# QitaoZhao/ContextAware-PoseFormer

Hardware: AMD Instinct MI355X
Metric: frames/sec (higher is better)
Workload: dtype f32; 1 GPU; configs[1]: batch 64/GPU hrnet_32 256x256 image + 17 kpts -> 17x3, PoseFormer lifter embed 128 levels 4, fp32 tensors, fp32 accumulation; 3x3 stride-1 convs from batch 5: each operand as two fp16 pieces under exact power-of-two block scales (to 2^-23), three piece products on the 16-bit matrix pipe -- same measured distance to fp64 as the direct fp32 MFMA kernel; Inf / NaN / |x| >= 1.5e23 give NaN; frames_per_gpu=64, parallelism=dp1 (independent frames, no collective), plan_flags=0

## Files before the change

contextaware-poseformer_amd/csrc/engine.cpp:

```cpp
#include <stdio.h>
#include <string.h>

#include <algorithm>
#include <vector>

#include "engine.h"

namespace capf {

#define HIP_TRY(expr)                                                                      \
    do {                                                                                   \
        hipError_t _e = (expr);                                                            \
        if (_e != hipSuccess) {                                                            \
            err = std::string(#expr) + ": " + hipGetErrorString(_e);                       \
            return CAPF_ERR_HIP;                                                           \
        }                                                                                  \
    } while (0)

Engine::ConvSrc Engine::conv_src(const Pack& pk) const {
    return {params[pk.w[0]].ptr, params[pk.bn.g].ptr, params[pk.bn.b].ptr, params[pk.bn.m].ptr, params[pk.bn.v].ptr, 1e-5f};
}

int Engine::repack(hipStream_t s, bool lifter_only) {
    for (const Param& p : params) {
// ... 20 lines not shown
        float* B = pack_arena + pk.b_off;
        if (pk.kind == CONV_BN) {
            if (lifter_only) continue;
            const ConvSrc c = conv_src(pk);
            if (pk.bf16) {
                HIP_TRY(launch_pack_conv_bf16(c.w, c.g, c.b, c.m, c.v, c.eps, W, B, pk.N, pk.Cin, pk.ks, pk.Kpad, s, f16()));
                if (pk.rh) HIP_TRY(launch_pack_conv_bf16_rh(c.w, c.g, c.b, c.m, c.v, c.eps, pack_arena + pk.rh_off, B, pk.N, pk.Cin, bf16_rh_width(pk.Cin), s, f16()));
                if (pk.ws) HIP_TRY(launch_pack_conv_bf16_ws(c.w, c.g, c.b, c.m, c.v, c.eps, pack_arena + pk.ws_off, B, pk.N, pk.Cin, s, f16()));
            } else if (pk.fast3x3) {
                if (!pk.wino_skip) HIP_TRY(launch_pack_conv_wino(c.w, c.g, c.b, c.m, c.v, c.eps, W, B, pk.N, pk.Cin, s, pk.Kpad == 18 * pk.Cin ? 43 : 23));
                HIP_TRY(launch_pack_conv(c.w, c.g, c.b, c.m, c.v, c.eps, pack_arena + pk.direct_off, B, pk.N, pk.Cin, pk.ks, pk.direct_Kpad, s));
                if (pk.x3)
                    HIP_TRY((plan.x3_h2 ? launch_pack_conv_f32h2 : launch_pack_conv_f32x3)(c.w, c.g, c.b, c.m, c.v, c.eps, pack_arena + pk.x3_off, B, pk.N, pk.Cin, s));
            } else {
                HIP_TRY(launch_pack_conv(c.w, c.g, c.b, c.m, c.v, c.eps, W, B, pk.N, pk.Cin, pk.ks, pk.Kpad, s));
            }
            continue;
        }
        int n0 = 0;
        for (int i = 0; i < pk.n_lin; ++i) {
            const int n = (int)params[pk.w[i]].shape[0];
            const float* w = params[pk.w[i]].ptr;
            if (pk.bf16)
                HIP_TRY(launch_pack_conv_bf16(w, nullptr, nullptr, nullptr, nullptr, 0.f, reinterpret_cast<unsigned short*>(W) + (size_t)n0 * pk.Kpad,
                                              nullptr, n, pk.K, 1, pk.Kpad, s, f16()));
            else if (pk.quad) HIP_TRY(launch_pack_linear_quad(w, W, n, pk.K, n0, pk.N, s));
            else HIP_TRY(launch_pack_linear(w, W + (size_t)n0 * pk.Kpad, n, pk.K, pk.Kpad, s));
            jobs.push_back(CopySegment{params[pk.b[i]].ptr, B + n0, n, 0});
            n0 += n;
        }
// ... 36 lines not shown
    GemmArgs a{};
    a.A = op.in[0] == -2 ? images : ptr(op.in[0]);
    if (pk.in_place) {
        a.Wp = params[pk.w[0]].ptr;
        a.bias = params[pk.b[0]].ptr;
    } else {
        a.Wp = pack_arena + pk.w_off;
        a.bias = pack_arena + pk.b_off;
    }
    a.res = op.res_param >= 0 ? params[op.res_param].ptr : ptr(op.aux);
    a.out = ptr(op.out);
    a.M = (int)(op.rows_per_frame * batch);
    a.N = op.N; a.K = op.K; a.Kpad = pk.Kpad;
    if (pk.rh) a.Wp2 = pack_arena + pk.rh_off;
    if (pk.ws || pk.x3) a.Wp3 = pack_arena + (pk.ws ? pk.ws_off : pk.x3_off);
    a.x3_h2 = pk.x3 && plan.x3_h2;
    if (a.x3_h2 && op.h2_utab >= 0 && utab_on_device) a.h2_utab = reinterpret_cast<const unsigned*>(pack_arena + utab_off) + op.h2_utab;
    const Family family = gemm_family(op, batch);
    if (pk.h2g && batch >= H2G_MIN_BATCH && family == Family::F32 && !op.pw_pair) a.Wh2 = pack_arena + pk.h2g_off;
    if (op.fast3x3 && family == Family::F32) {
        a.Wp = pack_arena + pk.direct_off;
        a.Kpad = pk.direct_Kpad;
    } else if (family == Family::F32_TILE && pk.wino_skip) {
        a.Wp = nullptr;
    }
    a.conv = op.conv;
    a.Cin = op.Cin; a.H = op.H; a.W = op.W; a.Ho = op.Ho; a.Wo = op.Wo;
    a.ks = op.ks; a.stride = op.stride; a.pad = op.pad;
    a.amap = op.amap; a.omap = op.omap; a.rmap = op.rmap;
    a.act = op.act;
// ... 18 lines not shown
        a.split_cnt = on_side_chain ? split_cnt_side : split_cnt;
        a.split_ws_elems = SPLIT_WS_ELEMS; a.split_cnt_elems = SPLIT_CNT_ELEMS;
    }
    if (op.ln.w >= 0) {
        a.ln_g = params[op.ln.w].ptr;
        a.ln_b = params[op.ln.b].ptr;
        a.ln_eps = op.eps;
    }
    return a;
}

Engine::FusedLaunch Engine::fused_at(int i, int batch, int last_op, bool bneck_only) const {
    const int n_all = (int)ops.size();
    if (i < 0 || i >= n_all) return {};
    const Op& o = ops[i];
    if (o.kind == OP_FORK) {
        if (!plan.use_bneck || !b16() || o.fork.lanes != 2 || o.region < 0) return {};
        const int j = regions[o.region].second;
        if (j != i + 4 || j + 1 >= last_op || j + 1 >= n_all) return {};
        int c1 = -1, c2 = -1, ds = -1;
        for (int k = i + 1; k < j; ++k) {
            const Op& g = ops[k];
            if (g.kind != OP_GEMM || !g.conv || g.bf16 != 1) return {};
            if (g.lane == 1) ds = k; else if (c1 < 0) c1 = k; else c2 = k;
        }
        const int c3 = j + 1;
        if (c1 < 0 || c2 < 0 || ds < 0 || ops[c3].kind != OP_GEMM || !ops[c3].conv || ops[c3].bf16 != 1) return {};
        if (ops[c2].in[0] != ops[c1].out || ops[ds].in[0] != ops[c1].in[0] || ops[c3].in[0] != ops[c2].out || ops[c3].aux != ops[ds].out) return {};
        if (ops[c1].rows_per_frame * batch < 65536) return {};
        if (!bneck0_bf16_ok(gemm_args(ops[c1], batch), gemm_args(ops[c2], batch), gemm_args(ops[ds], batch), gemm_args(ops[c3], batch))) return {};
// ... 6 lines not shown
                  o.rows_per_frame * batch >= 65536;
        for (const Op* g : {&o, &c2, &c3})
            ok = ok && g->kind == OP_GEMM && g->conv && g->bf16 == 1 && g->region == o.region && g->lane == o.lane && g->up_in < 0;
        if (ok && bneck1_bf16_ok(gemm_args(o, batch), gemm_args(c2, batch), gemm_args(c3, batch))) return {Fusion::BNECK1, 3, {i, i + 1, i + 2}};
    }
    if (bneck_only || !plan.use_pwchain || i + 1 >= last_op || i + 1 >= n_all) return {};
    const Op& b = ops[i + 1];
    if (!o.conv || b.kind != OP_GEMM || !b.conv || o.bf16 != b.bf16 || o.bf16 > 1 || b.in[0] != o.out || b.region != o.region || b.lane != o.lane) return {};
    if (o.bf16 && (fused_leader(i, batch, true).n || fused_at(i + 1, batch, last_op, true).n)) return {};
    const GemmArgs ga = gemm_args(o, batch), gb = gemm_args(b, batch);
    if (!(o.bf16 ? gemm_bf16_pwchain_ok(ga, gb) : gemm_f32_pwchain_ok(ga, gb))) return {};
    return {Fusion::PWCHAIN, 2, {i, i + 1}};
}

Engine::FusedLaunch Engine::fused_leader(int i, int batch, bool bneck_only) const {
    for (int f = i - 5; f <= i; ++f) {
        const FusedLaunch l = fused_at(f, batch, (int)ops.size(), bneck_only);
        for (int k = 0; k < l.n; ++k)
            if (l.m[k] == i) return l;
    }
    return {};
}

Engine::Family Engine::gemm_family(const Op& op, int batch) const {
    const bool tile = batch >= op.tile_lo && batch <= op.tile_hi;
    if (op.bf16) return op.bf16 == 2 ? Family::BF16_ROWS : tile ? Family::BF16_TILE : Family::BF16;
    if (tile) return Family::F32_TILE;
    return op.fast3x3 && batch >= plan.wino_min_batch && !packs[op.pack].wino_skip ? Family::WINO : Family::F32;
}

bool Engine::tile_takes(const Op& op, int batch) const {
// ... 160 lines not shown
            HIP_TRY(launch_mlp_chain(ptr(op.out), op.amap, (int)(op.rows_per_frame * batch), op.eps, w, s));
            break;
        }
        case OP_HEAD:
            HIP_TRY(launch_head(ptr(op.in[0]), params[op.ln.w].ptr, params[op.ln.b].ptr, op.eps, params[op.head.w].ptr,
                                params[op.head.b].ptr, out, (int)(op.rows_per_frame * batch), op.C, op.head.N, s));
            break;
        default: break;
    }
    return CAPF_OK;
}

int Engine::run_region_grouped(hipStream_t s, int batch, int region, LaunchLog* log, unsigned lane_mask) {
    auto mine = [&](const Op& op) { return ((lane_mask >> op.lane) & 1u) != 0; };
    auto groupable = [&](const Op& op, const GemmArgs& a) {
        if (op.kind != OP_GEMM) return false;
        switch (gemm_family(op, batch)) {
            case Family::BF16: return gemm_bf16_groupable(a);
            case Family::BF16_TILE: case Family::F32_TILE: return true;
            case Family::WINO: return gemm_wino_ok(a);
            case Family::F32: return gemm_f32_groupable(a);
            default: return false;
        }
    };
    for (const std::vector<int>& level : region_levels[region]) {
        for (Family pass : {Family::F32, Family::BF16_TILE, Family::BF16, Family::F32_TILE, Family::WINO}) {
            GemmArgs group[MAXG];
            int members[MAXG];
            int n = 0;
            auto flush = [&]() -> int {
                if (n == 0) return CAPF_OK;
// ... 62 lines not shown
    hipStream_t main_stream = s;
    if (plan.use_h2g && (batch >= H2G_MIN_BATCH || has_res_chain) && last_op > n_backbone_ops && !b16()) {
        const int rc = ensure_h2g_lifter(s);
        if (rc) return rc;
    }
    const bool grouped = (lanes == 2 || lanes == 3) && !ev;
    const bool par = lanes == 1 && !ev && !log && side[0];
    for (int oi = first_op; oi < last_op; ++oi) {
        const Op& op = ops[oi];
        s = (par && op.lane > 0) ? side[op.lane - 1] : main_stream;
        if (ev) HIP_TRY(hipEventRecord(ev[oi], s));
        if (const FusedLaunch f = ev ? FusedLaunch{} : fused_at(oi, batch, last_op); f.n) {
            const bool tap = debug || last_op < (int)ops.size();
            GemmArgs m[4];
            for (int k = 0; k < f.n; ++k) m[k] = gemm_args(ops[f.m[k]], batch);
            if (log) HIP_TRY(log->mark(s, f.m, f.n));
            if (f.kind == Fusion::BNECK0) HIP_TRY(launch_bneck0_bf16(m[0], m[1], m[2], m[3], tap, s));
            else if (f.kind == Fusion::BNECK1) HIP_TRY(launch_bneck1_bf16(m[0], m[1], m[2], tap, s));
            else if (op.bf16) HIP_TRY(launch_gemm_bf16_pwchain(m[0], m[1], s));
            else HIP_TRY(launch_gemm_f32_pwchain(m[0], m[1], s));
            oi = f.m[f.n - 1];
            continue;
        }
        switch (op.kind) {
            case OP_FORK: {
                if (grouped && regions[op.region].second <= last_op) {
                    const bool two = two_chains(op, batch) && !log && side[0];
                    if (two) {
                        HIP_TRY(hipEventRecord(events[op.fork.first_event], main_stream));
                        HIP_TRY(hipStreamWaitEvent(side[0], events[op.fork.first_event], 0));
// ... 884 lines not shown
    return capf::launch_keypoints_loss(pred, gt, validity, rows, dim, mode, threshold, loss, dpred,
                                       static_cast<hipStream_t>(stream)) == hipSuccess ? CAPF_OK : CAPF_ERR_HIP;
}

int capf_num_ops(const capf_handle* h) { return h ? (int)h->e.ops.size() : CAPF_ERR_INVALID; }

int capf_op_info(const capf_handle* h, int index, int batch, const char** name, const char** kernel, double* flops) {
    if (!h || index < 0 || index >= (int)h->e.ops.size() || batch <= 0) return CAPF_ERR_INVALID;
    const capf::Op& op = h->e.ops[index];
    if (name) *name = op.name.c_str();
    if (flops) *flops = op.flops_per_frame * batch;
    if (kernel) {
        const capf::Engine::FusedLaunch f = h->e.fused_leader(index, batch);
        *kernel = f.kind == capf::Engine::Fusion::BNECK0 ? capf::bneck0_bf16_kernel_name(h->e.f16())
                  : f.kind == capf::Engine::Fusion::BNECK1 ? capf::bneck1_bf16_kernel_name(h->e.f16())
                  : f.kind == capf::Engine::Fusion::PWCHAIN ? (op.bf16 ? capf::gemm_bf16_pwchain_kernel_name(h->e.f16()) : capf::gemm_f32_pwchain_kernel_name())
                  : h->e.op_route(op, batch).kernel;
    }
    return CAPF_OK;
}

int capf_op_executed_flops(const capf_handle* h, int index, int batch, double* flops) {
    if (!h || index < 0 || index >= (int)h->e.ops.size() || batch <= 0 || !flops) return CAPF_ERR_INVALID;
    *flops = h->e.op_route(h->e.ops[index], batch).flops;
    return CAPF_OK;
}

int capf_op_bytes(const capf_handle* h, int index, int batch, double* bytes) {
    if (!h || index < 0 || index >= (int)h->e.ops.size() || batch <= 0 || !bytes) return CAPF_ERR_INVALID;
    const capf::Engine& e = h->e;
    const capf::Op& op = e.ops[index];
    const double B = batch, act = op.bf16 ? 2.0 : 4.0;
    const double fact = op.feat_bf16 ? 2.0 : 4.0;
    const capf::Sampler& sm = op.smp;
    const capf::Attn& at = op.attn;
    double b = 0.0;
    switch (op.kind) {
        case capf::OP_GEMM: {
            const capf::Pack& pk = e.packs[op.pack];
            const double M = (double)op.rows_per_frame * B;
            const double in_elems = op.conv ? B * op.H * op.W * op.Cin : M * op.K;
            if (op.bf16 == 2) {
                b = in_elems * 2.0 + (double)pk.N * pk.K * 2.0 + (double)pk.N * 4.0 + M * op.N * (op.out_bf16 ? 2.0 : 4.0) +
                    (op.aux >= 0 ? M * op.N * 4.0 : 0.0);
                break;
            }
            b = in_elems * (op.conv && !op.bf16 ? 4.0 : act)
                + (double)pk.N * pk.K * (pk.bf16 ? 2.0 : 4.0) + (double)pk.N * 4.0
                + M * op.N * (op.st_f32 ? 4.0 + (op.sh >= 0 ? 2.0 : 0.0) : op.out_bf16 ? 2.0 : act)
                + ((op.aux >= 0 || op.res_param >= 0) ? M * op.N * (op.f32s ? 4.0 : act) : 0.0)
                + ((op.conv && op.up_in >= 0) ? B * op.up_H * op.up_W * op.N * act : 0.0);
            break;
        }
        case capf::OP_FUSE: {
            const double out = B * op.H * op.W * op.C;
            b = out * act + (op.sh >= 0 ? out * 2.0 : 0.0);
            for (int i = 0; i < op.n_in; ++i) b += out * act / (double)(1 << (2 * op.shift[i]));
            break;
        }
// ... 259 lines not shown
```

contextaware-poseformer_amd/csrc/engine.h:

```cpp
#pragma once
#include <hip/hip_runtime.h>
#include <stdint.h>

#include <array>
#include <map>
#include <string>
#include <vector>

#include "capf.h"
#include "kernels.h"

namespace capf {

struct Param {
    std::string name;
    int64_t shape[4] = {0, 0, 0, 0};
    int ndim = 0;
    int kind = 0;
    const float* ptr = nullptr;
    int64_t numel() const {
        int64_t n = 1;
        for (int i = 0; i < ndim; ++i) n *= shape[i];
        return n;
    }
// ... 21 lines not shown
    int n_lin = 0;
    BnRef bn;
    int N = 0, K = 0, Cin = 0, ks = 1;
    size_t w_off = 0, b_off = 0;
    int Kpad = 0;
    bool in_place = false;
    bool bf16 = false;
    bool quad = false;
    bool fast3x3 = false;
    bool wino_skip = false;
    size_t direct_off = 0; int direct_Kpad = 0;
    bool rh = false; size_t rh_off = 0; int rh_Kpad = 0;
    bool ws = false; size_t ws_off = 0;
    bool x3 = false; size_t x3_off = 0;
    bool h2g = false; size_t h2g_off = 0; int h2g_Kpad = 0;
    bool chain = false; size_t chain_off = 0;
};

struct LinearRef { int w = -1, b = -1, N = 0, K = 0; };
struct LnRef { int w = -1, b = -1; };
struct LifterMlp { LnRef norm2; LinearRef fc1, fc2; };
struct LifterAtt { LnRef norm1; LinearRef qkv, proj; LifterMlp mlp; };
struct LifterCtx {
    LnRef norm1;
    LinearRef aw, so, embed_proj[4];
    LifterMlp mlp;
    int ao_pack = -1;
    int tap_pos = -1, tap_idx = -1;
};
struct LifterSchema {
// ... 40 lines not shown
    Sampler smp;
    LinearRef coord;
    int pos = -1;
    LinearRef head;
    Attn attn;
    std::vector<ChainBlock> blocks;
    int lvlH[4] = {0, 0, 0, 0}, lvlW[4] = {0, 0, 0, 0}, lvlC[4] = {0, 0, 0, 0};
    int idx_lvl[4] = {-1, -1, -1, -1};
    int tap_pos = -1, tap_idx = -1;
    int pq[4] = {-1, -1, -1, -1};
    int pb[4] = {-1, -1, -1, -1};
    double flops_per_frame = 0.0;
    int bf16 = 0;
    int fast3x3 = 0;
    int pw_pair = 0;
    int tile_lo = 0, tile_hi = -1;
    int out_bf16 = 0;
    int h2_exps = -1, h2_role = 0, h2_peer = -1;
    long h2_utab = -1;
    int f32s = 0, st_f32 = 0, sh = -1;
    int feat_bf16 = 0;
    int bneck_c3 = -1;
    int lane = 0;
    int region = -1;
    int level = -1;
};

struct NamedTensor {
    int buf;
    int64_t shape[4];
// ... 144 lines not shown
    ConvSrc conv_src(const Pack& pk) const;
    int repack(hipStream_t s, bool lifter_only = false);
    int ensure_h2g_lifter(hipStream_t s);
    int run(hipStream_t s, int batch, int first_op, int last_op, hipEvent_t* ev = nullptr, LaunchLog* log = nullptr);
    int exec_op(const Op& op, hipStream_t s, int batch);
    bool skipped(const Op& op) const { return op.debug_only && !debug; }
    FuseSumArgs fuse_args(const Op& op, int batch) const;
    enum class Family { NONE = -1, F32, BF16, BF16_TILE, F32_TILE, WINO, BF16_ROWS };
    struct OpRoute { Family family; const char* kernel; double flops; };
    bool tile_takes(const Op& op, int batch) const;
    Family gemm_family(const Op& op, int batch) const;
    hipError_t launch_f32_tile(const GemmArgs* list, int n, hipStream_t s) const {
        return (plan.x3_h2 ? launch_gemm_f32h2_group : launch_gemm_f32x3_group)(list, n, s);
    }
    OpRoute op_route(const Op& op, int batch) const;
    enum class Fusion { NONE, BNECK0, BNECK1, PWCHAIN };
    struct FusedLaunch { Fusion kind = Fusion::NONE; int n = 0; int m[4] = {-1, -1, -1, -1}; };
    FusedLaunch fused_at(int i, int batch, int last_op, bool bneck_only = false) const;
    FusedLaunch fused_leader(int i, int batch, bool bneck_only = false) const;
    int run_region_grouped(hipStream_t s, int batch, int region, LaunchLog* log, unsigned lane_mask = ~0u);
    bool two_chains(const Op& fork_op, int batch) const { return lanes == 3 && fork_op.fork.lanes >= 2 && batch >= 16 && batch <= 128; }
    GemmArgs gemm_args(const Op& op, int batch, bool planes = true) const;

    int train_batch = 0;
    int64_t train_generation = 0;
    void invalidate_train() { train_batch = 0; ++train_generation; t_h2_base = nullptr; }
    int feat_batch = 0;
    void train_layout(int B, TrainLayout& L) const;
    size_t train_elems(int B) const;
    int forward_train(hipStream_t s, int B, const float* masks);
    int backward(hipStream_t s, int B, const float* dOut, float* flat_grad, const float* masks, float* const* dfeat = nullptr);
// ... 34 lines not shown
```

contextaware-poseformer_amd/csrc/igemm_f32_pwchain.hip:

```cpp
#include "kernels.h"

namespace capf {

typedef float f32x4 __attribute__((ext_vector_type(4)));
typedef float f32x16 __attribute__((ext_vector_type(16)));
typedef unsigned u32x4 __attribute__((ext_vector_type(4)));
typedef __amdgpu_buffer_rsrc_t rsrc_t;

template <int K1, int N1, int N2>
__global__ __launch_bounds__(256, 1) void igemm_f32_pwchain_kernel(GemmArgs p3, GemmArgs p1, int ntiles) {
#if defined(__HIP_DEVICE_COMPILE__)
    constexpr int NT1 = N1 / 32, NT2 = N2 / 32, ST1 = K1 / 8;
    constexpr int W3F = N1 * K1, W1F = N2 * N1;
    constexpr unsigned OOB = 0x80000000u;
    static_assert(K1 % 32 == 0 && N1 % 32 == 0 && N2 == 64, "whole 32-float sub-chunks; eight MFMA groups per sub-chunk of the second conv");
    constexpr int EPS = 36;
    extern __shared__ __attribute__((aligned(16))) float lds[];
    float* W3s = lds;
    float* W1s = lds + W3F;
    float* B3s = W1s + W1F;
    float* B1s = B3s + N1;
    const int tid = threadIdx.x, lane = tid & 63;
    const int wave = __builtin_amdgcn_readfirstlane(tid >> 6);

// ... 146 lines not shown
                for (int e = 0; e < 4; ++e) v[e] = relu_f(z[jn][4 * g + e] + bv[e]);
                *reinterpret_cast<f32x4*>(&ep[frow * EPS + 8 * g + 4 * fhalf]) = v;
            }
            __builtin_amdgcn_wave_barrier();
#pragma unroll
            for (int h = 0; h < 4; ++h) {
                const f32x4 v = *reinterpret_cast<const f32x4*>(&ep[(8 * h + er) * EPS + ec]);
                __builtin_amdgcn_raw_buffer_store_b128(__builtin_bit_cast(u32x4, v), rs_t,
                                                       m0 + 8 * h + er < p3.M ? (unsigned)((8 * h + er) * (int)s_t + 32 * jn + ec) * 4u : OOB, 0, 0);
            }
        }
    }
#endif
}

bool gemm_f32_pwchain_ok(const GemmArgs& a, const GemmArgs& b) {
    static const int on = [] { const char* e = diag_env("CAPF_PWCHAIN"); return e ? atoi(e) : 1; }();
    auto plain = [](const GemmArgs& g) {
        return g.conv && g.ks == 1 && g.stride == 1 && g.pad == 0 && g.K == g.Cin && g.Kpad == g.K && g.omap.G == 1 && (g.omap.S1 & 3) == 0 &&
               (g.omap.off & 3) == 0 && !g.rscale && !g.ln_g && g.splits <= 1 && g.act != ACT_GELU && !g.out_bf16;
    };
    if (!on || !plain(a) || !plain(b)) return false;
    if (a.K != 64 || a.N != 256 || b.K != 256 || b.N != 64 || b.res || a.M != b.M) return false;
    if (!a.res || !a.bias || !b.bias || a.act != ACT_RELU || b.act != ACT_RELU) return false;
    if (b.A != a.out + a.omap.off || a.omap.S1 != b.K) return false;
    if (a.rmap.G != 1 || (a.rmap.S1 & 3) || (a.rmap.off & 3)) return false;
    if ((long)a.omap.S1 * 32 * 4 >= (1L << 31) || (long)a.rmap.S1 * 32 * 4 >= (1L << 31)) return false;
    {
        auto overlaps = [](const float* p0, long n0, const float* p1, long n1) { return p0 < p1 + n1 && p1 < p0 + n0; };
        const float* bo = b.out + b.omap.off;
        const long bn = (long)(b.M - 1) * b.omap.S1 + b.N;
        if (overlaps(bo, bn, a.res + a.rmap.off, (long)(a.M - 1) * a.rmap.S1 + a.N)) return false;
        if (overlaps(bo, bn, a.A, (long)a.M * a.K)) return false;
    }
    return a.M >= 32 * 1024 * 4;
}

const char* gemm_f32_pwchain_kernel_name() { return "igemm_f32_pwchain<64,256,64>"; }

hipError_t launch_gemm_f32_pwchain(const GemmArgs& a, const GemmArgs& b, hipStream_t s) {
    if (!gemm_f32_pwchain_ok(a, b)) return hipErrorInvalidValue;
    const int ntiles = (a.M + 31) / 32;
    constexpr size_t lds_bytes = (size_t)(256 * 64 + 64 * 256 + 256 + 64 + 4 * 32 * 36) * 4;
    static DynLdsAttr attr_once;
    const hipError_t attr = attr_once.ensure(reinterpret_cast<const void*>(&igemm_f32_pwchain_kernel<64, 256, 64>), (int)lds_bytes);
    if (attr != hipSuccess) return attr;
    hipLaunchKernelGGL((igemm_f32_pwchain_kernel<64, 256, 64>), dim3(256), dim3(256), lds_bytes, s, a, b, ntiles);
    return hipGetLastError();
}

}
```

contextaware-poseformer_amd/csrc/kernels.h:

```cpp
#pragma once
#include <hip/hip_runtime.h>
#include <stdint.h>

#include <stdlib.h>

#include "relu.h"
#include "fmt16.h"
#include "capf.h"

namespace capf {

inline const char* diag_env(const char* name) {
#ifdef CAPF_DIAG
    return getenv(name);
#else
    (void)name;
    return nullptr;
#endif
}

struct BilinearCorner {
    int x0, y0;
    float wx1, wy1;
};
// ... 164 lines not shown
    return (double)rows * (double)a.omap.S1 * elem_bytes < 2.0e9 && (!a.res || (double)rows * (double)a.rmap.S1 * elem_bytes < 2.0e9);
}
bool gemm_f32_groupable(const GemmArgs& a);
bool gemm_f32_rows_splitk(const GemmArgs& a);
hipError_t launch_gemm_f32_group(const GemmArgs* list, int n, hipStream_t s);
enum class F32Path { PW, H2G, SPLITK_GROUP, ROWS_SPLITK, STEM_BF16, STEM_STREAM, SMALLC, TILE };
struct F32Route { F32Path path; int tile; };
F32Route gemm_f32_route(const GemmArgs& a);
const char* gemm_f32_kernel_name(const GemmArgs& a);
bool gemm_f32_pw_ok(const GemmArgs& a);
hipError_t launch_gemm_f32_pw(const GemmArgs& a, hipStream_t s);
const char* gemm_f32_pw_kernel_name();
bool gemm_f32_pwchain_ok(const GemmArgs& a, const GemmArgs& b);
hipError_t launch_gemm_f32_pwchain(const GemmArgs& a, const GemmArgs& b, hipStream_t s);
const char* gemm_f32_pwchain_kernel_name();
bool bneck0_bf16_ok(const GemmArgs& c1, const GemmArgs& c2, const GemmArgs& ds, const GemmArgs& c3);
hipError_t launch_bneck0_bf16(const GemmArgs& c1, const GemmArgs& c2, const GemmArgs& ds, const GemmArgs& c3, bool tap, hipStream_t s);
const char* bneck0_bf16_kernel_name(int f16 = 0);
bool bneck1_bf16_ok(const GemmArgs& c1, const GemmArgs& c2, const GemmArgs& c3);
hipError_t launch_bneck1_bf16(const GemmArgs& c1, const GemmArgs& c2, const GemmArgs& c3, bool tap, hipStream_t s);
const char* bneck1_bf16_kernel_name(int f16 = 0);
bool gemm_bf16_pwchain_ok(const GemmArgs& a, const GemmArgs& b);
hipError_t launch_gemm_bf16_pwchain(const GemmArgs& a, const GemmArgs& b, hipStream_t s);
const char* gemm_bf16_pwchain_kernel_name(int f16 = 0);

bool gemm_wino_ok(const GemmArgs& a);
hipError_t launch_gemm_wino(const GemmArgs& a, hipStream_t s);
hipError_t launch_gemm_wino_group(const GemmArgs* list, int n, hipStream_t s);
const char* gemm_wino_kernel_name(const GemmArgs& a);
hipError_t launch_pack_conv_wino(const float* w, const float* gamma, const float* beta, const float* mean, const float* var,
// ... 260 lines not shown
```

contextaware-poseformer_amd/csrc/plan.cpp:

```cpp
#include <limits.h>
#include <stdlib.h>

#include <algorithm>
#include <map>
#include <tuple>

#include "engine.h"

namespace capf {

static const int EXT_IMAGES = -2;

static size_t round64(size_t n) { return (n + 63) / 64 * 64; }
static int round32(int n) { return (n + 31) / 32 * 32; }
static int round64(int n) { return (n + 63) / 64 * 64; }

int Engine::add_param(const std::string& name, int kind, std::initializer_list<int64_t> shape) {
    auto it = param_index.find(name);
    if (it != param_index.end()) return it->second;
    Param p;
    p.name = name;
    p.kind = kind;
    p.ndim = (int)shape.size();
    int i = 0;
// ... 177 lines not shown
}

static void bneck1_mark(Engine& e, int c1) {
    if (!e.plan.use_bneck || !e.b16() || c1 + 2 >= (int)e.ops.size()) return;
    const Op &o1 = e.ops[c1], &o2 = e.ops[c1 + 1], &o3 = e.ops[c1 + 2];
    if (o1.kind != OP_GEMM || o2.kind != OP_GEMM || o3.kind != OP_GEMM || o1.Cin != 256 || o1.N != 64 || o2.ks != 3 || o2.stride != 1 || o3.N != 256 || o3.aux != o1.in[0]) return;
    for (int b : {o1.in[0], o1.out, o2.out, o3.out}) {
        if (b < 0) continue;
        e.bufs[b].def_op = std::min(e.bufs[b].def_op, c1);
        e.bufs[b].last_op = std::max(e.bufs[b].last_op, c1 + 2);
    }
    e.ops[c1].bneck_c3 = c1 + 2;
    e.ops[c1 + 1].bneck_c3 = c1 + 2;
}

static Tensor hr_bottleneck(Engine& e, const std::string& p, const Tensor& x, int planes, bool down) {
    const int fork_at = (int)e.ops.size();
    if (down) e.fork(2);
    Tensor y = e.conv_bn(p + ".conv1", p + ".bn1", x, planes, 1, 1, ACT_RELU, nullptr);
    y = e.conv_bn(p + ".conv2", p + ".bn2", y, planes, 3, 1, ACT_RELU, nullptr);
    Tensor r = x;
    if (down) {
        e.set_lane(1);
        r = e.conv_bn(p + ".downsample.0", p + ".downsample.1", x, planes * 4, 1, 1, ACT_NONE, nullptr);
        e.join();
    }
    Tensor out = e.conv_bn(p + ".conv3", p + ".bn3", y, planes * 4, 1, 1, ACT_RELU, &r);
    if (down) bneck0_mark(e, fork_at);
    else bneck1_mark(e, fork_at);
    return out;
}

static void hr_module(Engine& e, const std::string& p, std::vector<Tensor>& xs, int n_out, int blocks,
                      std::vector<Tensor>* branch_out) {
    const int nb = (int)xs.size();
    std::vector<Tensor> br(nb);
    e.fork(nb);
    for (int i = 0; i < nb; ++i) {
        e.set_lane(i);
        Tensor y = xs[i];
        for (int k = 0; k < blocks; ++k)
            y = hr_basic_block(e, p + ".branches." + std::to_string(i) + "." + std::to_string(k), y);
        br[i] = y;
// ... 112 lines not shown
    for (int li = 0; li < 4; ++li) {
        for (int k = 0; k < nblk[li]; ++k) {
            const std::string p = R + ".layer" + std::to_string(li + 1) + "." + std::to_string(k);
            const int st = (k == 0) ? strides[li] : 1;
            const int fork_at = (int)ops.size();
            if (k == 0) fork(2);
            Tensor y = conv_bn(p + ".conv1", p + ".bn1", x, planes[li], 1, 1, ACT_RELU, nullptr);
            y = conv_bn(p + ".conv2", p + ".bn2", y, planes[li], 3, st, ACT_RELU, nullptr);
            Tensor r = x;
            if (k == 0) {
                set_lane(1);
                r = conv_bn(p + ".downsample.0", p + ".downsample.1", x, planes[li] * 4, 1, st, ACT_NONE, nullptr);
                join();
            }
            x = conv_bn(p + ".conv3", p + ".bn3", y, planes[li] * 4, 1, 1, ACT_RELU, &r);
            if (k == 0 && st == 1) bneck0_mark(*this, fork_at);
            if (k > 0) bneck1_mark(*this, fork_at);
        }
        c[li] = x;
    }
    const std::string G = "backbone.global_net";
    Tensor fms[4];
    for (int i = 0; i < 4; ++i) {
        const Tensor& src = c[3 - i];
        const std::string lp = G + ".laterals." + std::to_string(i);
        if (i > 0 && b16() && plan.use_upadd) {
            const std::string upn = G + ".upsamples." + std::to_string(i - 1);
            Tensor t = conv_bn(upn + ".1", upn + ".2", fms[i - 1], 256, 1, 1, ACT_NONE, nullptr);
            ops.back().flops_per_frame *= 4.0;
            fms[i] = conv_bn(lp + ".0", lp + ".1", src, 256, 1, 1, ACT_RELU, nullptr);
            Op& lop = ops.back();
// ... 745 lines not shown
            pk.direct_off = off;
            off += round64((size_t)pk.N * pk.direct_Kpad);
        }
        if (pk.rh) {
            pk.rh_off = off;
            off += round64(((size_t)pk.N * pk.rh_Kpad + 1) / 2);
        }
        if (pk.ws) {
            pk.ws_off = off;
            off += round64(((size_t)bf16_ws_pack_elems(pk.N, pk.Cin) + 1) / 2);
        }
        if (pk.x3) {
            pk.x3_off = off;
            off += round64(((size_t)(plan.x3_h2 ? f32h2_pack_elems(pk.N, pk.Cin) : f32x3_pack_elems(pk.N, pk.Cin)) + 1) / 2);
        }
        pk.b_off = off;
        off += round64((size_t)pk.N);
    }
    for (Pack& pk : packs)
        if (pk.h2g) {
            pk.h2g_off = off;
            off += round64((size_t)f32h2_gemm_pack_elems(pk.N, pk.h2g_Kpad));
            if (pk.chain) {
                pk.chain_off = off;
                off += round64((size_t)f32h2_gemm_pack_elems(pk.N, pk.h2g_Kpad));
            }
        }
    {
        size_t nseg = 0;
        for (const Pack& pk : packs)
// ... 15 lines not shown
```

Baseline: 9650 frames/s.

## Fuse bottleneck downsample shortcut into fp32 pointwise chain kernel

Adds a fused fp32 kernel for the first bottleneck block (stride 1, 64->256 channels). It computes the downsample 1x1 conv, conv3 with the residual add and ReLU, and the next block's 1x1 conv in one persistent launch. The downsample weights are prepacked into MFMA fragment order and streamed through a register ring, and both other weight sets stay in LDS. This removes the downsample output round trip through global memory and two launches, at the cost of a large, register-heavy kernel that runs one block per CU and forces the fork region to be serialised on the main stream.

Result: no change. 9722 frames/s (median of 6 runs) (+0.7%).

```diff
diff --git a/contextaware-poseformer_amd/csrc/engine.cpp b/contextaware-poseformer_amd/csrc/engine.cpp
--- a/contextaware-poseformer_amd/csrc/engine.cpp
+++ b/contextaware-poseformer_amd/csrc/engine.cpp
@@ -58,6 +58,7 @@
                     HIP_TRY((plan.x3_h2 ? launch_pack_conv_f32h2 : launch_pack_conv_f32x3)(c.w, c.g, c.b, c.m, c.v, c.eps, pack_arena + pk.x3_off, B, pk.N, pk.Cin, s));
             } else {
                 HIP_TRY(launch_pack_conv(c.w, c.g, c.b, c.m, c.v, c.eps, W, B, pk.N, pk.Cin, pk.ks, pk.Kpad, s));
+                if (pk.frag) HIP_TRY(launch_pwchain_sc_pack(W, pack_arena + pk.frag_off, pk.N, pk.Kpad, s));
             }
             continue;
         }
@@ -124,6 +125,7 @@
     a.N = op.N; a.K = op.K; a.Kpad = pk.Kpad;
     if (pk.rh) a.Wp2 = pack_arena + pk.rh_off;
     if (pk.ws || pk.x3) a.Wp3 = pack_arena + (pk.ws ? pk.ws_off : pk.x3_off);
+    if (pk.frag) a.Wp3 = pack_arena + pk.frag_off;
     a.x3_h2 = pk.x3 && plan.x3_h2;
     if (a.x3_h2 && op.h2_utab >= 0 && utab_on_device) a.h2_utab = reinterpret_cast<const unsigned*>(pack_arena + utab_off) + op.h2_utab;
     const Family family = gemm_family(op, batch);
@@ -172,6 +174,14 @@
     const int n_all = (int)ops.size();
     if (i < 0 || i >= n_all) return {};
     const Op& o = ops[i];
+    if (o.kind == OP_FORK && !b16()) {
+        if (bneck_only || !plan.use_pwchain || debug || o.fork.lanes != 2 || o.region < 0) return {};
+        const int j = regions[o.region].second, ds = i + 3, c3 = i + 5, n1 = i + 6;
+        if (j != i + 4 || n1 >= last_op || n1 >= n_all || !ops[ds].pw_sc || !ops[c3].pw_pair || !ops[n1].pw_pair) return {};
+        if (ops[c3].aux != ops[ds].out || ops[n1].in[0] != ops[c3].out || ops[ds].in[0] != ops[i + 1].in[0]) return {};
+        if (!gemm_f32_pwchain_sc_ok(gemm_args(ops[ds], batch), gemm_args(ops[c3], batch), gemm_args(ops[n1], batch))) return {};
+        return {Fusion::PWCHAIN_SC, 3, {ds, c3, n1}};
+    }
     if (o.kind == OP_FORK) {
         if (!plan.use_bneck || !b16() || o.fork.lanes != 2 || o.region < 0) return {};
         const int j = regions[o.region].second;
@@ -208,7 +218,7 @@
 }
 
 Engine::FusedLaunch Engine::fused_leader(int i, int batch, bool bneck_only) const {
-    for (int f = i - 5; f <= i; ++f) {
+    for (int f = i - 6; f <= i; ++f) {
         const FusedLaunch l = fused_at(f, batch, (int)ops.size(), bneck_only);
         for (int k = 0; k < l.n; ++k)
             if (l.m[k] == i) return l;
@@ -399,7 +409,7 @@
 int Engine::run_region_grouped(hipStream_t s, int batch, int region, LaunchLog* log, unsigned lane_mask) {
     auto mine = [&](const Op& op) { return ((lane_mask >> op.lane) & 1u) != 0; };
     auto groupable = [&](const Op& op, const GemmArgs& a) {
-        if (op.kind != OP_GEMM) return false;
+        if (op.kind != OP_GEMM || op.pw_sc) return false;
         switch (gemm_family(op, batch)) {
             case Family::BF16: return gemm_bf16_groupable(a);
             case Family::BF16_TILE: case Family::F32_TILE: return true;
@@ -492,6 +502,23 @@
             const bool tap = debug || last_op < (int)ops.size();
             GemmArgs m[4];
             for (int k = 0; k < f.n; ++k) m[k] = gemm_args(ops[f.m[k]], batch);
+            if (f.kind == Fusion::PWCHAIN_SC) {
+                if (grouped) {
+                    const int rc = run_region_grouped(main_stream, batch, op.region, log, ~0x2u);
+                    if (rc) return rc;
+                } else {
+                    for (int k = oi + 1; k < regions[op.region].second; ++k) {
+                        if (ops[k].lane == 1) continue;
+                        if (log) HIP_TRY(log->mark(main_stream, &k, 1));
+                        const int rc = exec_op(ops[k], main_stream, batch);
+                        if (rc) return rc;
+                    }
+                }
+                if (log) HIP_TRY(log->mark(main_stream, f.m, f.n));
+                HIP_TRY(launch_gemm_f32_pwchain_sc(m[0], m[1], m[2], main_stream));
+                oi = f.m[f.n - 1];
+                continue;
+            }
             if (log) HIP_TRY(log->mark(s, f.m, f.n));
             if (f.kind == Fusion::BNECK0) HIP_TRY(launch_bneck0_bf16(m[0], m[1], m[2], m[3], tap, s));
             else if (f.kind == Fusion::BNECK1) HIP_TRY(launch_bneck1_bf16(m[0], m[1], m[2], tap, s));
@@ -1406,6 +1433,7 @@
         const capf::Engine::FusedLaunch f = h->e.fused_leader(index, batch);
         *kernel = f.kind == capf::Engine::Fusion::BNECK0 ? capf::bneck0_bf16_kernel_name(h->e.f16())
                   : f.kind == capf::Engine::Fusion::BNECK1 ? capf::bneck1_bf16_kernel_name(h->e.f16())
+                  : f.kind == capf::Engine::Fusion::PWCHAIN_SC ? capf::gemm_f32_pwchain_sc_kernel_name()
                   : f.kind == capf::Engine::Fusion::PWCHAIN ? (op.bf16 ? capf::gemm_bf16_pwchain_kernel_name(h->e.f16()) : capf::gemm_f32_pwchain_kernel_name())
                   : h->e.op_route(op, batch).kernel;
     }
@@ -1435,6 +1463,12 @@
             if (op.bf16 == 2) {
                 b = in_elems * 2.0 + (double)pk.N * pk.K * 2.0 + (double)pk.N * 4.0 + M * op.N * (op.out_bf16 ? 2.0 : 4.0) +
                     (op.aux >= 0 ? M * op.N * 4.0 : 0.0);
+                break;
+            }
+            const capf::Engine::FusedLaunch fl = op.pw_sc || op.pw_pair ? e.fused_leader(index, batch) : capf::Engine::FusedLaunch{};
+            const bool sc = fl.kind == capf::Engine::Fusion::PWCHAIN_SC;
+            if (sc && index != fl.m[2]) {
+                b = in_elems * 4.0 + (double)pk.N * pk.K * 4.0 + (double)pk.N * 4.0 + (index == fl.m[1] ? M * op.N * 4.0 : 0.0);
                 break;
             }
             b = in_elems * (op.conv && !op.bf16 ? 4.0 : act)
diff --git a/contextaware-poseformer_amd/csrc/engine.h b/contextaware-poseformer_amd/csrc/engine.h
--- a/contextaware-poseformer_amd/csrc/engine.h
+++ b/contextaware-poseformer_amd/csrc/engine.h
@@ -59,6 +59,7 @@
     bool ws = false; size_t ws_off = 0;
     bool x3 = false; size_t x3_off = 0;
     bool h2g = false; size_t h2g_off = 0; int h2g_Kpad = 0;
+    bool frag = false; size_t frag_off = 0;
     bool chain = false; size_t chain_off = 0;
 };
 
@@ -129,6 +130,7 @@
     int bf16 = 0;
     int fast3x3 = 0;
     int pw_pair = 0;
+    int pw_sc = 0;
     int tile_lo = 0, tile_hi = -1;
     int out_bf16 = 0;
     int h2_exps = -1, h2_role = 0, h2_peer = -1;
@@ -303,7 +305,7 @@
         return (plan.x3_h2 ? launch_gemm_f32h2_group : launch_gemm_f32x3_group)(list, n, s);
     }
     OpRoute op_route(const Op& op, int batch) const;
-    enum class Fusion { NONE, BNECK0, BNECK1, PWCHAIN };
+    enum class Fusion { NONE, BNECK0, BNECK1, PWCHAIN, PWCHAIN_SC };
     struct FusedLaunch { Fusion kind = Fusion::NONE; int n = 0; int m[4] = {-1, -1, -1, -1}; };
     FusedLaunch fused_at(int i, int batch, int last_op, bool bneck_only = false) const;
     FusedLaunch fused_leader(int i, int batch, bool bneck_only = false) const;
diff --git a/contextaware-poseformer_amd/csrc/igemm_f32_pwchain.hip b/contextaware-poseformer_amd/csrc/igemm_f32_pwchain.hip
--- a/contextaware-poseformer_amd/csrc/igemm_f32_pwchain.hip
+++ b/contextaware-poseformer_amd/csrc/igemm_f32_pwchain.hip
@@ -1,3 +1,5 @@
+#include <type_traits>
+
 #include "kernels.h"
 
 namespace capf {
@@ -184,7 +186,236 @@
 #endif
 }
 
-bool gemm_f32_pwchain_ok(const GemmArgs& a, const GemmArgs& b) {
+template <int K1, int N1, int N2>
+__global__ __launch_bounds__(256, 1) void igemm_f32_pwchain_sc_kernel(GemmArgs p3, GemmArgs p1, GemmArgs pd, int ntiles) {
+#if defined(__HIP_DEVICE_COMPILE__)
+    constexpr int NT1 = N1 / 32, NT2 = N2 / 32, ST1 = K1 / 8;
+    constexpr int W3F = N1 * K1, W1F = N2 * N1;
+    constexpr int NG = ST1 * NT1, WR = 8;
+    static_assert(NG % WR == 0, "the ring wraps around from one tile to the next: group g lives in slot g % WR");
+    constexpr unsigned OOB = 0x80000000u;
+    static_assert(K1 % 32 == 0 && N1 % 32 == 0 && N2 == 64, "whole 32-float sub-chunks; eight MFMA groups per sub-chunk of the second conv");
+    constexpr int EPS = 36;
+    extern __shared__ __attribute__((aligned(16))) float lds[];
+    float* W3s = lds;
+    float* W1s = lds + W3F;
+    float* B3s = W1s + W1F;
+    float* BDs = B3s + N1;
+    float* B1s = BDs + N1;
+    const int tid = threadIdx.x, lane = tid & 63;
+    const int wave = __builtin_amdgcn_readfirstlane(tid >> 6);
+
+    auto stage = [&](const float* W, float* dst, auto n_c, auto k_c) {
+        constexpr int N = decltype(n_c)::value, K = decltype(k_c)::value, qpr = K / 4;
+        static_assert(N * qpr % 256 == 0, "whole rounds of the block");
+        f32x4 v[N * qpr / 256];
+#pragma unroll
+        for (int it = 0; it < N * qpr / 256; ++it) {
+            const int i = it * 256 + tid, n = i / qpr, q = i - n * qpr;
+            v[it] = *reinterpret_cast<const f32x4*>(W + (size_t)n * K + q * 4);
+        }
+#pragma unroll
+        for (int it = 0; it < N * qpr / 256; ++it) {
+            const int i = it * 256 + tid, n = i / qpr, q = i - n * qpr;
+            const int sub = q >> 3, qq = q & 7;
+            *reinterpret_cast<f32x4*>(dst + (size_t)sub * N * 32 + n * 32 + ((qq ^ ((n >> 1) & 7)) * 4)) = v[it];
+        }
+    };
+    stage(p3.Wp, W3s, std::integral_constant<int, N1>{}, std::integral_constant<int, K1>{});
+    stage(p1.Wp, W1s, std::integral_constant<int, N2>{}, std::integral_constant<int, N1>{});
+    for (int i = tid; i < N1; i += 256) { B3s[i] = p3.bias[i]; BDs[i] = pd.bias[i]; }
+    for (int i = tid; i < N2; i += 256) B1s[i] = p1.bias[i];
+    __syncthreads();
+
+    float* ep = B1s + N2 + wave * (32 * EPS);
+    const int frow = lane & 31, fhalf = lane >> 5, fsw = (frow >> 1) & 7;
+    const int er = lane >> 3, ec = (lane & 7) * 4;
+    const int gw = blockIdx.x * 4 + wave, nw = gridDim.x * 4;
+    const long s_a = p3.K, s_x = pd.K, s_y = p3.omap.S1, s_t = p1.omap.S1;
+
+    const float* bq = &B3s[4 * fhalf];
+    float* ep_acc = &ep[frow * EPS + 4 * fhalf];
+    float* ep_row = &ep[er * EPS + ec];
+    const float *w3q[4], *w1q[4];
+#pragma unroll
+    for (int q = 0; q < 4; ++q) {
+        w3q[q] = &W3s[frow * 32 + ((q * 2 + fhalf) ^ fsw) * 4];
+        w1q[q] = &W1s[frow * 32 + ((q * 2 + fhalf) ^ fsw) * 4];
+    }
+    f32x4 a1[ST1];
+    f32x4 xf[ST1];
+    f32x4 wd[WR];
+    auto request_a = [&](int tile) {
+        const bool live = tile < ntiles;
+        const rsrc_t rs = __builtin_amdgcn_make_buffer_rsrc((void*)(p3.A + (live ? (long)tile * 32 : 0) * s_a), 0, 0x7FFFFF00u, 0x00020000);
+        const unsigned row = live && tile * 32 + frow < p3.M ? (unsigned)(frow * (int)s_a + fhalf * 4) * 4u : OOB;
+#pragma unroll
+        for (int st = 0; st < ST1; ++st) a1[st] = __builtin_bit_cast(f32x4, __builtin_amdgcn_raw_buffer_load_b128(rs, row, st * 32, 0));
+    };
+    auto request_x = [&](int tile) {
+        const rsrc_t rx = __builtin_amdgcn_make_buffer_rsrc((void*)(pd.A + (long)tile * 32 * s_x), 0, 0x7FFFFF00u, 0x00020000);
+        const unsigned row = tile * 32 + frow < p3.M ? (unsigned)(frow * (int)s_x + fhalf * 4) * 4u : OOB;
+#pragma unroll
+        for (int st = 0; st < ST1; ++st) xf[st] = __builtin_bit_cast(f32x4, __builtin_amdgcn_raw_buffer_load_b128(rx, row, st * 32, 0));
+    };
+    const rsrc_t rs_w = __builtin_amdgcn_make_buffer_rsrc((void*)pd.Wp3, 0, (unsigned)(N1 * K1 * 4), 0x00020000);
+    auto request_wd = [&](int g) {
+        wd[g % WR] = __builtin_bit_cast(f32x4, __builtin_amdgcn_raw_buffer_load_b128(rs_w, (unsigned)(g * 256 + lane * 4) * 4u, 0, 0));
+    };
+
+    int tile = gw;
+    request_a(tile);
+#pragma unroll
+    for (int g = 0; g < WR; ++g) request_wd(g);
+    for (; tile < ntiles; tile += nw) {
+        const long m0 = (long)tile * 32;
+        f32x16 y[NT1];
+#pragma unroll
+        for (int j = 0; j < NT1; ++j)
+#pragma unroll
+            for (int r = 0; r < 16; ++r) y[j][r] = 0.f;
+        auto w3_frag = [&](int st, int j) {
+            return *reinterpret_cast<const f32x4*>(w3q[st & 3] + ((st >> 2) * (N1 * 32) + 32 * j * 32));
+        };
+        {
+            f32x4 bf = w3_frag(0, 0);
+#pragma unroll
+            for (int st = 0; st < ST1; ++st)
+#pragma unroll
+                for (int j = 0; j < NT1; ++j) {
+                    const int jn = j + 1 < NT1 ? j + 1 : 0, sn = j + 1 < NT1 ? st : (st + 1 < ST1 ? st + 1 : st);
+                    const f32x4 nx = w3_frag(sn, jn);
+#pragma unroll
+                    for (int e = 0; e < 4; ++e) y[j] = __builtin_amdgcn_mfma_f32_32x32x2f32(bf[e], a1[st][e], y[j], 0, 0, 0);
+                    bf = nx;
+                    if (st == 0 && j == 0) request_x(tile);
+                    __builtin_amdgcn_sched_barrier(0);
+                }
+        }
+        const rsrc_t rs_y = __builtin_amdgcn_make_buffer_rsrc((void*)(p3.out + m0 * s_y + p3.omap.off), 0, 0x7FFFFF00u, 0x00020000);
+        f32x16 acc_d[NT1];
+        f32x4 ev0, ev1, evo;
+        auto epi_step = [&](int j, int piece, int step) {
+            if (piece < 4) {
+                const int g = piece;
+                if (step == 0) {
+                    if (g == 0) __builtin_amdgcn_wave_barrier();
+                    ev0 = *reinterpret_cast<const f32x4*>(bq + (32 * j + 8 * g));
+                    ev1 = *reinterpret_cast<const f32x4*>(bq + (N1 + 32 * j + 8 * g));
+                } else if (step >= 2) {
+#pragma unroll
+                    for (int e = 2 * (step - 2); e < 2 * (step - 2) + 2; ++e) {
+                        float t = (y[j][4 * g + e] + ev0[e]) + (acc_d[j][4 * g + e] + ev1[e]);
+                        t = relu_f(t);
+                        y[j][4 * g + e] = t;
+                        evo[e] = t;
+                    }
+                    if (step == 3) {
+                        *reinterpret_cast<f32x4*>(ep_acc + 8 * g) = evo;
+                        if (g == 3) __builtin_amdgcn_wave_barrier();
+                    }
+                }
+            } else {
+                const int h = (piece - 4) * 2;
+                if (step == 0) {
+                    ev0 = *reinterpret_cast<const f32x4*>(ep_row + 8 * h * EPS);
+                    ev1 = *reinterpret_cast<const f32x4*>(ep_row + 8 * (h + 1) * EPS);
+                } else if (step >= 2) {
+                    const int hh = h + step - 2;
+                    __builtin_amdgcn_raw_buffer_store_b128(__builtin_bit_cast(u32x4, step == 2 ? ev0 : ev1), rs_y,
+                                                           m0 + 8 * hh + er < p3.M ? (unsigned)((8 * hh + er) * (int)s_y + ec) * 4u : OOB, 32 * j * 4, 0);
+                }
+            }
+        };
+#pragma unroll
+        for (int j = 0; j < NT1; ++j)
+#pragma unroll
+            for (int r = 0; r < 16; ++r) acc_d[j][r] = 0.f;
+#pragma unroll
+        for (int st = 0; st < ST1; ++st)
+#pragma unroll
+            for (int j = 0; j < NT1; ++j) {
+                const int g = st * NT1 + j;
+                const f32x4 bf = wd[g % WR];
+#pragma unroll
+                for (int e = 0; e < 4; ++e) {
+                    acc_d[j] = __builtin_amdgcn_mfma_f32_32x32x2f32(bf[e], xf[st][e], acc_d[j], 0, 0, 0);
+                    if (g > NG - NT1 && g - (NG - NT1 + 1) < 6) epi_step(0, g - (NG - NT1 + 1), e);
+                    if (e == 3) request_wd((g + WR) % NG);
+                    __builtin_amdgcn_sched_barrier(0);
+                }
+            }
+        f32x16 z[NT2];
+#pragma unroll
+        for (int jn = 0; jn < NT2; ++jn)
+#pragma unroll
+            for (int r = 0; r < 16; ++r) z[jn][r] = 0.f;
+        auto w1_frag = [&](int j, int g, int jn) {
+            return *reinterpret_cast<const f32x4*>(w1q[g] + (j * (N2 * 32) + 32 * jn * 32));
+        };
+        {
+            f32x4 bf = w1_frag(0, 0, 0);
+#pragma unroll
+            for (int j = 0; j < NT1; ++j)
+#pragma unroll
+                for (int g = 0; g < 4; ++g)
+#pragma unroll
+                    for (int jn = 0; jn < NT2; ++jn) {
+                        const bool last_n = jn + 1 == NT2, last_g = g == 3;
+                        const int n2 = last_n ? 0 : jn + 1, g2 = last_n ? (last_g ? 0 : g + 1) : g,
+                                  j2 = last_n && last_g ? (j + 1 < NT1 ? j + 1 : j) : j;
+                        const f32x4 nx = w1_frag(j2, g2, n2);
+#pragma unroll
+                        for (int e = 0; e < 4; ++e) {
+                            z[jn] = __builtin_amdgcn_mfma_f32_32x32x2f32(bf[e], y[j][4 * g + e], z[jn], 0, 0, 0);
+                            if (j + 1 < NT1 && g * NT2 + jn < 6) epi_step(j + 1, g * NT2 + jn, e);
+                            if (j == NT1 / 2 && g == 0 && jn == 0 && e == 1) request_a(tile + nw);
+                            __builtin_amdgcn_sched_barrier(0);
+                        }
+                        bf = nx;
+                    }
+        }
+        const rsrc_t rs_t = __builtin_amdgcn_make_buffer_rsrc((void*)(p1.out + m0 * s_t + p1.omap.off), 0, 0x7FFFFF00u, 0x00020000);
+#pragma unroll
+        for (int jn = 0; jn < NT2; ++jn) {
+            __builtin_amdgcn_wave_barrier();
+#pragma unroll
+            for (int g = 0; g < 4; ++g) {
+                const f32x4 bv = *reinterpret_cast<const f32x4*>(bq + (2 * N1 + 32 * jn + 8 * g));
+                f32x4 v;
+#pragma unroll
+                for (int e = 0; e < 4; ++e) v[e] = relu_f(z[jn][4 * g + e] + bv[e]);
+                *reinterpret_cast<f32x4*>(ep_acc + 8 * g) = v;
+            }
+            __builtin_amdgcn_wave_barrier();
+#pragma unroll
+            for (int h = 0; h < 4; ++h) {
+                const f32x4 v = *reinterpret_cast<const f32x4*>(ep_row + 8 * h * EPS);
+                __builtin_amdgcn_raw_buffer_store_b128(__builtin_bit_cast(u32x4, v), rs_t,
+                                                       m0 + 8 * h + er < p3.M ? (unsigned)((8 * h + er) * (int)s_t + ec) * 4u : OOB, 32 * jn * 4, 0);
+            }
+        }
+    }
+#endif
+}
+
+__global__ void pwchain_sc_pack_kernel(const float* __restrict__ W, float* __restrict__ dst, int N, int K) {
+    const int i = blockIdx.x * blockDim.x + threadIdx.x;
+    if (i >= N * K / 4) return;
+    const int lane = i & 63, g = i >> 6, nt = N / 32;
+    const int st = g / nt, j = g - st * nt;
+    *reinterpret_cast<f32x4*>(dst + (size_t)i * 4) =
+        *reinterpret_cast<const f32x4*>(W + (size_t)(32 * j + (lane & 31)) * K + 8 * st + 4 * (lane >> 5));
+}
+
+hipError_t launch_pwchain_sc_pack(const float* W, float* dst, int N, int K, hipStream_t s) {
+    if (N % 32 || K % 8) return hipErrorInvalidValue;
+    const int n = N * K / 4;
+    hipLaunchKernelGGL(pwchain_sc_pack_kernel, dim3((n + 255) / 256), dim3(256), 0, s, W, dst, N, K);
+    return hipGetLastError();
+}
+
+static bool pwchain_pair_ok(const GemmArgs& a, const GemmArgs& b, bool res_read) {
     static const int on = [] { const char* e = diag_env("CAPF_PWCHAIN"); return e ? atoi(e) : 1; }();
     auto plain = [](const GemmArgs& g) {
         return g.conv && g.ks == 1 && g.stride == 1 && g.pad == 0 && g.K == g.Cin && g.Kpad == g.K && g.omap.G == 1 && (g.omap.S1 & 3) == 0 &&
@@ -200,11 +431,13 @@
         auto overlaps = [](const float* p0, long n0, const float* p1, long n1) { return p0 < p1 + n1 && p1 < p0 + n0; };
         const float* bo = b.out + b.omap.off;
         const long bn = (long)(b.M - 1) * b.omap.S1 + b.N;
-        if (overlaps(bo, bn, a.res + a.rmap.off, (long)(a.M - 1) * a.rmap.S1 + a.N)) return false;
+        if (res_read && overlaps(bo, bn, a.res + a.rmap.off, (long)(a.M - 1) * a.rmap.S1 + a.N)) return false;
         if (overlaps(bo, bn, a.A, (long)a.M * a.K)) return false;
     }
     return a.M >= 32 * 1024 * 4;
 }
+
+bool gemm_f32_pwchain_ok(const GemmArgs& a, const GemmArgs& b) { return pwchain_pair_ok(a, b, true); }
 
 const char* gemm_f32_pwchain_kernel_name() { return "igemm_f32_pwchain<64,256,64>"; }
 
@@ -219,4 +452,33 @@
     return hipGetLastError();
 }
 
-}
+bool gemm_f32_pwchain_sc_ok(const GemmArgs& ds, const GemmArgs& a, const GemmArgs& b) {
+    if (!a.res || !ds.out || !ds.A || !ds.Wp3 || !ds.bias) return false;
+    if (!pwchain_pair_ok(a, b, false)) return false;
+    const bool plain = ds.conv && ds.ks == 1 && ds.stride == 1 && ds.pad == 0 && ds.K == ds.Cin && ds.Kpad == ds.K && ds.omap.G == 1 && !ds.rscale &&
+                       !ds.ln_g && ds.splits <= 1 && !ds.out_bf16 && !ds.res;
+    if (!plain || ds.K != 64 || ds.N != 256 || ds.act != ACT_NONE || ds.M != a.M) return false;
+    if (a.res + a.rmap.off != ds.out + ds.omap.off || a.rmap.S1 != ds.omap.S1) return false;
+    {
+        auto overlaps = [](const float* p0, long n0, const float* p1, long n1) { return p0 < p1 + n1 && p1 < p0 + n0; };
+        const long xn = (long)ds.M * ds.K;
+        if (overlaps(b.out + b.omap.off, (long)(b.M - 1) * b.omap.S1 + b.N, ds.A, xn)) return false;
+        if (overlaps(a.out + a.omap.off, (long)(a.M - 1) * a.omap.S1 + a.N, ds.A, xn)) return false;
+    }
+    return true;
+}
+
+const char* gemm_f32_pwchain_sc_kernel_name() { return "igemm_f32_pwchain_sc<64,256,64>"; }
+
+hipError_t launch_gemm_f32_pwchain_sc(const GemmArgs& ds, const GemmArgs& a, const GemmArgs& b, hipStream_t s) {
+    if (!gemm_f32_pwchain_sc_ok(ds, a, b)) return hipErrorInvalidValue;
+    const int ntiles = (a.M + 31) / 32;
+    constexpr size_t lds_bytes = (size_t)(256 * 64 + 64 * 256 + 256 + 256 + 64 + 4 * 32 * 36) * 4;
+    static DynLdsAttr attr_once;
+    const hipError_t attr = attr_once.ensure(reinterpret_cast<const void*>(&igemm_f32_pwchain_sc_kernel<64, 256, 64>), (int)lds_bytes);
+    if (attr != hipSuccess) return attr;
+    hipLaunchKernelGGL((igemm_f32_pwchain_sc_kernel<64, 256, 64>), dim3(256), dim3(256), lds_bytes, s, a, b, ds, ntiles);
+    return hipGetLastError();
+}
+
+}
diff --git a/contextaware-poseformer_amd/csrc/kernels.h b/contextaware-poseformer_amd/csrc/kernels.h
--- a/contextaware-poseformer_amd/csrc/kernels.h
+++ b/contextaware-poseformer_amd/csrc/kernels.h
@@ -202,6 +202,10 @@
 bool gemm_f32_pwchain_ok(const GemmArgs& a, const GemmArgs& b);
 hipError_t launch_gemm_f32_pwchain(const GemmArgs& a, const GemmArgs& b, hipStream_t s);
 const char* gemm_f32_pwchain_kernel_name();
+bool gemm_f32_pwchain_sc_ok(const GemmArgs& ds, const GemmArgs& a, const GemmArgs& b);
+hipError_t launch_gemm_f32_pwchain_sc(const GemmArgs& ds, const GemmArgs& a, const GemmArgs& b, hipStream_t s);
+const char* gemm_f32_pwchain_sc_kernel_name();
+hipError_t launch_pwchain_sc_pack(const float* W, float* dst, int N, int K, hipStream_t s);
 bool bneck0_bf16_ok(const GemmArgs& c1, const GemmArgs& c2, const GemmArgs& ds, const GemmArgs& c3);
 hipError_t launch_bneck0_bf16(const GemmArgs& c1, const GemmArgs& c2, const GemmArgs& ds, const GemmArgs& c3, bool tap, hipStream_t s);
 const char* bneck0_bf16_kernel_name(int f16 = 0);
diff --git a/contextaware-poseformer_amd/csrc/plan.cpp b/contextaware-poseformer_amd/csrc/plan.cpp
--- a/contextaware-poseformer_amd/csrc/plan.cpp
+++ b/contextaware-poseformer_amd/csrc/plan.cpp
@@ -215,6 +215,18 @@
     e.ops[c1 + 1].bneck_c3 = c1 + 2;
 }
 
+static void pwchain_sc_mark(Engine& e, int fork) {
+    if (e.b16() || fork + 6 != (int)e.ops.size()) return;
+    const int c1 = fork + 1, ds = fork + 3, c3 = fork + 5;
+    Op& od = e.ops[ds];
+    const Op &o1 = e.ops[c1], &o3 = e.ops[c3];
+    if (e.ops[fork].kind != OP_FORK || e.ops[fork + 4].kind != OP_JOIN || od.kind != OP_GEMM || !od.conv || od.ks != 1 || od.stride != 1) return;
+    if (od.Cin != 64 || od.N != 256 || od.act != ACT_NONE || od.in[0] != o1.in[0] || o3.aux != od.out || o3.Cin != 64 || o3.N != 256 || o3.ks != 1) return;
+    if (od.in[0] >= 0) e.bufs[od.in[0]].last_op = std::max(e.bufs[od.in[0]].last_op, c3 + 1);
+    od.pw_sc = 1;
+    e.packs[od.pack].frag = true;
+}
+
 static Tensor hr_bottleneck(Engine& e, const std::string& p, const Tensor& x, int planes, bool down) {
     const int fork_at = (int)e.ops.size();
     if (down) e.fork(2);
@@ -227,7 +239,7 @@
         e.join();
     }
     Tensor out = e.conv_bn(p + ".conv3", p + ".bn3", y, planes * 4, 1, 1, ACT_RELU, &r);
-    if (down) bneck0_mark(e, fork_at);
+    if (down) bneck0_mark(e, fork_at), pwchain_sc_mark(e, fork_at);
     else bneck1_mark(e, fork_at);
     return out;
 }
@@ -370,7 +382,7 @@
                 join();
             }
             x = conv_bn(p + ".conv3", p + ".bn3", y, planes[li] * 4, 1, 1, ACT_RELU, &r);
-            if (k == 0 && st == 1) bneck0_mark(*this, fork_at);
+            if (k == 0 && st == 1) bneck0_mark(*this, fork_at), pwchain_sc_mark(*this, fork_at);
             if (k > 0) bneck1_mark(*this, fork_at);
         }
         c[li] = x;
@@ -1146,6 +1158,10 @@
             pk.x3_off = off;
             off += round64(((size_t)(plan.x3_h2 ? f32h2_pack_elems(pk.N, pk.Cin) : f32x3_pack_elems(pk.N, pk.Cin)) + 1) / 2);
         }
+        if (pk.frag) {
+            pk.frag_off = off;
+            off += round64((size_t)pk.N * pk.Kpad);
+        }
         pk.b_off = off;
         off += round64((size_t)pk.N);
     }
```
